# Yoshiki172/Deep-Learning-based-RGBA-Image-Compression-with-Masked-Window-based-Attention

Hardware: AMD Instinct MI355X
Metric: MPixels/sec encode+decode, 256×256 RGBA batch; bpp & PSNR parity vs reference (higher is better)
Workload: dtype bf16; 1 GPU; AutoEncoderRGB_Journal forward encode+decode (BASELINE config 2), 256x256 RGBA; global_batch=8, per_gpu_batch=8, height=256, width=256, parallelism=replicas1, hip_graph=True, tile_cache=profiles/tune_fwd_bf16_b8_256.json

## Files before the change

### deep-learning-based-rgba-image-compression-with-masked-window-based-attention_amd/csrc/fused.hip

```cpp
#include <cstdlib>

#include "common.h"

namespace rgbac {

constexpr int kRuMaxGroups = 4;

struct RuGroup {
  const bf16_t* x; long long ldx;
  const bf16_t* w1; const bf16_t* w2; const bf16_t* w3;
  int kp1, kp2, kp3;
  const float* b1; const float* b2; const float* b3;
  bf16_t* out; long long ldo;
};
struct RuArgsDev {
  int batch, H, W, ngroups;
  int stagger;
  RuGroup g[kRuMaxGroups];
  const bf16_t* gw;
  const float* gb;
  const bf16_t* gid; long long ldid;
  unsigned* flags;
  unsigned* timeout;
};
// ... 750 lines not shown
  for (int j = 0; j < 3; ++j) b2v[j] = *reinterpret_cast<const float4*>(bs + 96 + 48 * wn + 16 * j + 4 * fq);
#pragma unroll
  for (int j = 0; j < 3; ++j) {
    const int n = 48 * wn + 16 * j + 4 * fq;
    const float4 bb = b2v[j];
#pragma unroll
    for (int i = 0; i < 4; ++i) {
      const int p = (4 * wm + i) * TX + fr;
      float v[4];
      ru_act4<RB>(v, acc2[j][i], bb);
      Elem<bf16_t>::st4(reinterpret_cast<bf16_t*>(&T2[p * TROW + n * 2]), v);
    }
  }
  RU_T(5);
  __syncthreads();
  RU_T(6);

  f32x4 acc3[6][4];
#pragma unroll
  for (int j = 0; j < 6; ++j)
#pragma unroll
    for (int i = 0; i < 4; ++i) acc3[j][i] = f32x4{0.f, 0.f, 0.f, 0.f};
  const unsigned char* const t2l = T2 + (4 * wm * TX + fr) * TROW + fq * 16;
#pragma unroll
  for (int ks = 0; ks < NK3; ++ks) {
    uint4 bv[4];
#pragma unroll
    for (int i = 0; i < 4; ++i) bv[i] = *reinterpret_cast<const uint4*>(t2l + i * TX * TROW + ks * 64);
#pragma unroll
    for (int j = 0; j < 6; ++j)
#pragma unroll
      for (int i = 0; i < 4; ++i) mma_step<bf16_t>(acc3[j][i], w3r[ks % R3][j], bv[i]);
    if (ks + R3 < NK3) {
#pragma unroll
      for (int j = 0; j < 6; ++j) w3r[ks % R3][j] = W3[(j * NK3 + ks + R3) * 64];
    }
  }
  if constexpr (RB != 0) load_res();
  float4 b3v[6];
#pragma unroll
  for (int j = 0; j < 6; ++j) b3v[j] = *reinterpret_cast<const float4*>(bs + 192 + 96 * wn + 16 * j + 4 * fq);
  __syncthreads();
#pragma unroll
  for (int i = 0; i < 4; ++i) {
    const int p = (4 * wm + i) * TX + fr;
#pragma unroll
    for (int j = 0; j < 6; ++j) {
      const int n = 96 * wn + 16 * j + 4 * fq;
      const float4 bb = b3v[j];
      const uint2 rr = res[i][j];
      float v[4];
      v[0] = acc3[j][i][0] + bb.x + bf2f(rr.x & 0xFFFF);
      v[1] = acc3[j][i][1] + bb.y + bf2f(rr.x >> 16);
      v[2] = acc3[j][i][2] + bb.z + bf2f(rr.y & 0xFFFF);
      v[3] = acc3[j][i][3] + bb.w + bf2f(rr.y >> 16);
      if (!RB) gelu4_fast(v);
      Elem<bf16_t>::st4(reinterpret_cast<bf16_t*>(OT + p * ORW + n * 2), v);
    }
  }
  __syncthreads();
  if constexpr (GATE) {
    if (blockIdx.z == 1) {
      ru_gate_tile(args, OT, tile, b, y0, x0, wn, wm, fr, fq, lane);
      return;
    }
  }
#pragma unroll
  for (int u = 0; u < TY * TX * 24 / NTH; ++u) {
    const int c = tid + NTH * u, p = c / 24, q = c - (c / 24) * 24;
    const long long pix = (long long)(b * args.H + y0 + p / TX) * args.W + x0 + p % TX;
    const uint4 v = *reinterpret_cast<const uint4*>(OT + p * ORW + q * 16);
    if constexpr (GATE) st16_wt(g.out + pix * g.ldo + q * 8, v);
    else *reinterpret_cast<uint4*>(g.out + pix * g.ldo + q * 8) = v;
  }
  if constexpr (GATE) {
    asm volatile("s_waitcnt vmcnt(0)" ::: "memory");
    __syncthreads();
    if (tid == 0)
      __hip_atomic_store(&args.flags[tile], 1u, __ATOMIC_RELAXED, __HIP_MEMORY_SCOPE_AGENT);
  }
  RU_T(7);
}
#undef RU_T

}

using namespace rgbac;

#ifdef RGBAC_RU_TIMING
extern "C" int rgbac_debug_ru_times(unsigned long long* host, int nblocks) {
  if (nblocks > 8192) nblocks = 8192;
  if (hipMemcpyFromSymbol(host, HIP_SYMBOL(g_ru_t), (size_t)nblocks * 16 * 8) != hipSuccess) return 1;
  return hipMemcpyFromSymbol(host + (size_t)nblocks * 16, HIP_SYMBOL(g_ru_w), (size_t)nblocks * 2 * 8) ==
                 hipSuccess ? 0 : 1;
}
#endif

extern "C" int rgbac_residual_unit(const rgbac_ru_args* args, int ngroups, void* stream) {
  return rgbac_residual_unit_ex(args, ngroups, 0, stream);
}

extern "C" int rgbac_residual_unit_ex(const rgbac_ru_args* args, int ngroups, int kind,
                                      void* stream) {
  RGBAC_REQUIRE(args != nullptr && ngroups >= 1 && ngroups <= kRuMaxGroups, "groups");
  const rgbac_ru_args* a = args;
  RGBAC_REQUIRE(a->dtype == RGBAC_BF16, "the fused residual unit is bf16 only");
  RGBAC_REQUIRE(kind == 0 || kind == 1, "kind: 0 = ResidualUnit, 1 = ResBlock");
  RGBAC_REQUIRE(a->channels == 192 || a->channels == 80, "fused units support C = 192 or 80");
  RGBAC_REQUIRE(a->batch > 0 && a->h > 0 && a->w > 0 && a->h % 8 == 0 && a->w % 8 == 0,
                "H and W must be positive multiples of 8");
  RuArgsDev d{};
  d.batch = a->batch; d.H = a->h; d.W = a->w; d.ngroups = ngroups;
  static const int stagger_env = [] {
    const char* e = getenv("RGBAC_RU_STAGGER");
    return e ? atoi(e) : 0;
  }();
  d.stagger = stagger_env;
  for (int i = 0; i < ngroups; ++i) {
    const rgbac_ru_args* q = &args[i];
    RGBAC_REQUIRE(q->dtype == a->dtype && q->channels == a->channels && q->batch == a->batch &&
                      q->h == a->h && q->w == a->w, "grouped units must share the geometry");
    RGBAC_REQUIRE(q->x && q->out && q->w1 && q->w2 && q->w3 && q->b1 && q->b2 && q->b3,
                  "null pointer");
    RGBAC_REQUIRE(q->x != q->out, "out must not alias x (the halo is read by other tiles)");
    RGBAC_REQUIRE(q->x_ldc >= a->channels && q->x_ldc % 8 == 0 && q->out_ldc >= a->channels &&
                      q->out_ldc % 4 == 0, "strides");
    if (a->channels == 192 && q->w1_kpad != 0)
      RGBAC_REQUIRE(q->w1_kpad >= 192 && q->w2_kpad >= 896 && q->w3_kpad >= 96 &&
                        q->w1_kpad % 8 == 0 && q->w2_kpad % 8 == 0 && q->w3_kpad % 8 == 0,
                    "packed weight k_pad (w1 >= 192, w2 >= 896 zero-padded, w3 >= 96)");
    RGBAC_REQUIRE(((uintptr_t)q->x % 16) == 0 && ((uintptr_t)q->w1 % 16) == 0 &&
                      ((uintptr_t)q->w2 % 16) == 0 && ((uintptr_t)q->w3 % 16) == 0,
                  "16-byte alignment");
    RuGroup& g = d.g[i];
    g.x = (const bf16_t*)q->x; g.ldx = q->x_ldc;
    g.w1 = (const bf16_t*)q->w1; g.w2 = (const bf16_t*)q->w2; g.w3 = (const bf16_t*)q->w3;
    g.kp1 = q->w1_kpad; g.kp2 = q->w2_kpad; g.kp3 = q->w3_kpad;
    g.b1 = q->b1; g.b2 = q->b2; g.b3 = q->b3;
    g.out = (bf16_t*)q->out; g.ldo = q->out_ldc;
  }
  hipStream_t st = reinterpret_cast<hipStream_t>(stream);
  if (a->channels == 80) {
    const long long tiles = (long long)a->batch * (a->h / 8) * (a->w / 8);
    RGBAC_REQUIRE(tiles < (1ll << 31), "too many tiles");
    const int ncu = device_cus();
    long long gx = ncu / ngroups;
    if (gx < 1) gx = 1;
    const char* dual_env = getenv("RGBAC_RU_SMALL_DUAL");
    const bool dual = (tiles > gx && !(dual_env && dual_env[0] == '0')) || (dual_env && dual_env[0] == '2');
    if (dual) {
      if (gx > (tiles + 1) / 2) gx = (tiles + 1) / 2;
      if (kind) hipLaunchKernelGGL((ru_small_kernel<1, 2>), dim3((unsigned)gx, 1, ngroups), dim3(512), 0, st, d);
      else hipLaunchKernelGGL((ru_small_kernel<0, 2>), dim3((unsigned)gx, 1, ngroups), dim3(512), 0, st, d);
    } else {
      if (gx > tiles) gx = tiles;
      if (kind) hipLaunchKernelGGL((ru_small_kernel<1, 1>), dim3((unsigned)gx, 1, ngroups), dim3(256), 0, st, d);
      else hipLaunchKernelGGL((ru_small_kernel<0, 1>), dim3((unsigned)gx, 1, ngroups), dim3(256), 0, st, d);
    }
    return check_launch("ru_small_kernel");
  }
  if (a->w1_kpad == 0) {
    RGBAC_REQUIRE(a->h % 8 == 0 && a->w % 16 == 0, "the streamed unit needs H % 8 == 0, W % 16 == 0");
    for (int i = 0; i < ngroups; ++i)
      RGBAC_REQUIRE(args[i].w1_kpad == 0 && args[i].w2_kpad == 0 && args[i].w3_kpad == 0 &&
                        ((uintptr_t)args[i].b1 % 16) == 0 && ((uintptr_t)args[i].b2 % 16) == 0 &&
                        ((uintptr_t)args[i].b3 % 16) == 0 && args[i].out_ldc % 8 == 0 &&
                        ((uintptr_t)args[i].out % 16) == 0,
                    "grouped units must all be fragment-major (16-B aligned biases and out rows)");
    const long long tiles = (long long)a->batch * (a->h / 8) * (a->w / 16);
    RGBAC_REQUIRE(tiles < (1ll << 31), "too many tiles");
    for (int i = 0; i < ngroups; ++i)
      RGBAC_REQUIRE((long long)a->batch * a->h * a->w * args[i].x_ldc < (1ll << 31),
                    "the streamed unit addresses x with 32-bit element offsets");
    if (kind) hipLaunchKernelGGL((ru_stream_kernel<1, 8>), dim3((unsigned)tiles, 1, ngroups), dim3(256), 0, st, d);
    else hipLaunchKernelGGL((ru_stream_kernel<0, 8>), dim3((unsigned)tiles, 1, ngroups), dim3(256), 0, st, d);
    return check_launch("ru_stream_kernel");
  }
  static const int wide_env = [] {
    const char* e = getenv("RGBAC_RU_TILE");
    return (e && e[0] == '8') ? 0 : 1;
  }();
  if (wide_env && a->w % 16 == 0) {
    const long long tiles = (long long)a->batch * (a->h / 8) * (a->w / 16);
    RGBAC_REQUIRE(tiles < (1ll << 31), "too many tiles");
    if (kind) hipLaunchKernelGGL((ru_fused_kernel<192, 96, 8, 16, 2, 1>), dim3((unsigned)tiles, 1, ngroups),
                                 dim3(256), 0, st, d);
    else hipLaunchKernelGGL((ru_fused_kernel<192, 96, 8, 16, 2>), dim3((unsigned)tiles, 1, ngroups),
                            dim3(256), 0, st, d);
  } else {
    const long long tiles = (long long)a->batch * (a->h / 8) * (a->w / 8);
    RGBAC_REQUIRE(tiles < (1ll << 31), "too many tiles");
    if (kind) hipLaunchKernelGGL((ru_fused_kernel<192, 96, 8, 8, 3, 1>), dim3((unsigned)tiles, 1, ngroups),
                                 dim3(256), 0, st, d);
    else hipLaunchKernelGGL((ru_fused_kernel<192, 96, 8, 8, 3>), dim3((unsigned)tiles, 1, ngroups),
                            dim3(256), 0, st, d);
  }
  return check_launch("ru_fused_kernel");
}

extern "C" int rgbac_residual_unit_gate(const rgbac_ru_args* args, const void* gate_w,
                                        const float* gate_b, const void* ident, int64_t ident_ldc,
                                        uint32_t* flags, int64_t nflags, void* stream) {
  RGBAC_REQUIRE(args != nullptr && gate_w && gate_b && ident && flags, "null pointer");
  const rgbac_ru_args* a = args;
  RGBAC_REQUIRE(a->dtype == RGBAC_BF16 && a->channels == 192,
                "the gated unit pair is bf16, C = 192 only");
  RGBAC_REQUIRE(a->batch > 0 && a->h > 0 && a->w > 0 && a->h % 8 == 0 && a->w % 16 == 0,
                "the gated unit pair needs H % 8 == 0, W % 16 == 0");
  const long long tiles = (long long)a->batch * (a->h / 8) * (a->w / 16);
  RGBAC_REQUIRE(tiles < (1ll << 31) && nflags >= tiles + 1,
                "flags: one zeroed word per 8 x 16 tile plus the timeout word (the last)");
  RGBAC_REQUIRE(((uintptr_t)flags % 4) == 0 && ((uintptr_t)gate_w % 16) == 0 &&
                    ((uintptr_t)gate_b % 16) == 0 && ((uintptr_t)ident % 8) == 0 &&
                    ident_ldc >= 192 && ident_ldc % 4 == 0,
                "gate operand alignment / stride");
  RGBAC_REQUIRE((long long)a->batch * a->h * a->w * ident_ldc < (1ll << 31) ||
                    ident_ldc > 0, "identity stride");
  RuArgsDev d{};
  d.batch = a->batch; d.H = a->h; d.W = a->w; d.ngroups = 2;
  for (int i = 0; i < 2; ++i) {
    const rgbac_ru_args* q = &args[i];
    RGBAC_REQUIRE(q->dtype == a->dtype && q->channels == 192 && q->batch == a->batch &&
                      q->h == a->h && q->w == a->w, "both units must share the geometry");
    RGBAC_REQUIRE(q->x && q->out && q->w1 && q->w2 && q->w3 && q->b1 && q->b2 && q->b3,
                  "null pointer");
    RGBAC_REQUIRE(q->x != q->out && q->out != ident, "out must alias neither x nor the identity");
    RGBAC_REQUIRE(q->w1_kpad == 0 && q->w2_kpad == 0 && q->w3_kpad == 0,
                  "fragment-major packs only (the streamed unit)");
    RGBAC_REQUIRE(q->x_ldc >= 192 && q->x_ldc % 8 == 0 && q->out_ldc >= 192 &&
                      q->out_ldc % 8 == 0, "strides");
    RGBAC_REQUIRE(((uintptr_t)q->x % 16) == 0 && ((uintptr_t)q->w1 % 16) == 0 &&
                      ((uintptr_t)q->w2 % 16) == 0 && ((uintptr_t)q->w3 % 16) == 0 &&
                      ((uintptr_t)q->b1 % 16) == 0 && ((uintptr_t)q->b2 % 16) == 0 &&
                      ((uintptr_t)q->b3 % 16) == 0 && ((uintptr_t)q->out % 16) == 0,
                  "16-byte alignment");
    RGBAC_REQUIRE((long long)a->batch * a->h * a->w * q->x_ldc < (1ll << 31),
                  "the streamed unit addresses x with 32-bit element offsets");
    RuGroup& g = d.g[i];
    g.x = (const bf16_t*)q->x; g.ldx = q->x_ldc;
    g.w1 = (const bf16_t*)q->w1; g.w2 = (const bf16_t*)q->w2; g.w3 = (const bf16_t*)q->w3;
    g.b1 = q->b1; g.b2 = q->b2; g.b3 = q->b3;
    g.out = (bf16_t*)q->out; g.ldo = q->out_ldc;
  }
  d.gw = (const bf16_t*)gate_w; d.gb = gate_b;
  d.gid = (const bf16_t*)ident; d.ldid = ident_ldc;
  d.flags = flags; d.timeout = flags + (nflags - 1);
  hipStream_t st = reinterpret_cast<hipStream_t>(stream);
  hipLaunchKernelGGL((ru_stream_kernel<0, 8, true>), dim3((unsigned)tiles, 1, 2), dim3(256), 0, st, d);
  return check_launch("ru_stream_kernel");
}
```

### deep-learning-based-rgba-image-compression-with-masked-window-based-attention_amd/rgbac/_lib.py

```python
import ctypes
import os

import torch

_HERE = os.path.dirname(os.path.abspath(__file__))
LIB_PATH = os.environ.get("RGBAC_LIB_PATH") or os.path.join(_HERE, "librgbac_hip.so")

F32, BF16 = 0, 1
ACT = dict(none=0, gelu=1, relu=2, lrelu=3, tanh_half=4, gate=5, gdn=6, igdn=7, masksel=8,
           gauss=9, sqbwd=10, dgelu=11, dlrelu=12)
CONV, CONVT_S2, SUBPEL2 = 0, 1, 2


class Src(ctypes.Structure):
    _fields_ = [("ptr", ctypes.c_void_p), ("ldc", ctypes.c_int64),
                ("channels", ctypes.c_int32), ("_pad", ctypes.c_int32)]


class ConvArgs(ctypes.Structure):
    _fields_ = [
        ("dtype", ctypes.c_int32), ("mode", ctypes.c_int32),
        ("batch", ctypes.c_int32), ("in_h", ctypes.c_int32), ("in_w", ctypes.c_int32),
        ("ksize", ctypes.c_int32), ("stride", ctypes.c_int32),
        ("nsrc", ctypes.c_int32), ("src", Src * 3),
# ... 5 lines not shown
        ("out_coff", ctypes.c_int32), ("act", ctypes.c_int32),
        ("act_param", ctypes.c_float), ("square_input", ctypes.c_int32),
        ("res0", ctypes.c_void_p), ("res0_ldc", ctypes.c_int64),
        ("res1", ctypes.c_void_p), ("res1_ldc", ctypes.c_int64),
        ("res2", ctypes.c_void_p), ("res2_ldc", ctypes.c_int64),
        ("sel", ctypes.c_void_p),
        ("tile", ctypes.c_int32), ("ksplit", ctypes.c_int32),
        ("workspace", ctypes.c_void_p),
        ("aux0", ctypes.c_void_p), ("aux1", ctypes.c_void_p), ("partial", ctypes.c_void_p),
        ("zout", ctypes.c_void_p), ("zout_ldc", ctypes.c_int64),
        ("tile_counters", ctypes.c_void_p),
    ]


class WgradArgs(ctypes.Structure):
    _fields_ = [
        ("dtype", ctypes.c_int32),
        ("batch", ctypes.c_int32), ("grid_h", ctypes.c_int32), ("grid_w", ctypes.c_int32),
        ("g", ctypes.c_void_p), ("g_ldc", ctypes.c_int64), ("g_channels", ctypes.c_int32),
        ("in_h", ctypes.c_int32), ("in_w", ctypes.c_int32), ("ksize", ctypes.c_int32),
        ("stride", ctypes.c_int32), ("pad", ctypes.c_int32),
        ("nsrc", ctypes.c_int32), ("cin_pad", ctypes.c_int32),
        ("src", Src * 3),
        ("square_input", ctypes.c_int32),
        ("n_pad", ctypes.c_int32), ("k_pad", ctypes.c_int32),
        ("nsplit", ctypes.c_int32),
        ("partial", ctypes.c_void_p), ("bias_partial", ctypes.c_void_p),
    ]


class RuArgs(ctypes.Structure):
    _fields_ = [
        ("dtype", ctypes.c_int32), ("channels", ctypes.c_int32), ("batch", ctypes.c_int32),
        ("h", ctypes.c_int32), ("w", ctypes.c_int32), ("_pad0", ctypes.c_int32),
        ("x", ctypes.c_void_p), ("x_ldc", ctypes.c_int64),
        ("w1", ctypes.c_void_p), ("w2", ctypes.c_void_p), ("w3", ctypes.c_void_p),
        ("w1_kpad", ctypes.c_int32), ("w2_kpad", ctypes.c_int32), ("w3_kpad", ctypes.c_int32),
        ("_pad1", ctypes.c_int32),
        ("b1", ctypes.c_void_p), ("b2", ctypes.c_void_p), ("b3", ctypes.c_void_p),
        ("out", ctypes.c_void_p), ("out_ldc", ctypes.c_int64),
    ]


class RansDecoderState(ctypes.Structure):
    _fields_ = [("state", ctypes.c_uint64), ("data", ctypes.c_void_p), ("size", ctypes.c_int64),
                ("pos", ctypes.c_int64)]


_VP, _I32, _I64, _F = ctypes.c_void_p, ctypes.c_int, ctypes.c_int64, ctypes.c_float
_D = ctypes.c_double
SIGNATURES = {
    "rgbac_abi_version": [],
    "rgbac_last_error": [],
    "rgbac_conv2d": [ctypes.POINTER(ConvArgs), _VP],
    "rgbac_conv_num_tiles": [],
    "rgbac_conv_tile_weight_layout": [ctypes.c_int],
    "rgbac_conv2d_grouped": [ctypes.c_void_p, _I32, _VP],
    "rgbac_conv2d_grouped_part": [ctypes.c_void_p, _I32, _I32, _VP],
    "rgbac_conv_max_groups": [],
    "rgbac_timer_create": [ctypes.POINTER(ctypes.c_void_p)],
    "rgbac_timer_record": [_VP, _VP],
    "rgbac_timer_elapsed_ms": [_VP, _VP, ctypes.POINTER(ctypes.c_float)],
    "rgbac_timer_destroy": [_VP],
    "rgbac_winattn_core": [_I32, _I32, _I32, _I32, _I32, _I32, _I32, _I32, _I32, _F,
                           _VP, _I64, _VP, _VP, _VP, _I64, _VP, _VP],
    "rgbac_winattn_core_ex": [_I32, _I32, _I32, _I32, _I32, _I32, _I32, _I32, _I32, _F,
                              _VP, _I64, _VP, _VP, _VP, _I64, _VP, _VP, _I32, _I32, _VP],
    "rgbac_gaussian_slice": [_I32, _I64, _I32, _VP, _I64, _VP, _I64, _VP, _I64, _VP,
                             _VP, _I64, _VP, _VP, _VP],
    "rgbac_eb_forward": [_I32, _I64, _I32, _VP, _I64, _VP, _VP, _VP, _I64, _VP, _VP, _VP],
    "rgbac_reduce_blocks": [_I64],
    "rgbac_finalize": [_I32, _I32, _I32, _I32, _I32, _I32, _VP, _VP, _I64, _VP, _VP, _I32,
                       _VP, _I32, _VP, _VP, _VP],
    "rgbac_finalize_blocks": [_I32, _I32],
    "rgbac_finalize_ex": [_I32, _I32, _I32, _I32, _I32, _I32, _VP, _VP, _I64, _VP, _VP, _I32,
                          _VP, _I32, _VP, _VP, _VP, _VP],
    "rgbac_forward_prologue": [_I32, _I32, _I32, _I32, _I32, _VP, _VP, _I64, _VP, _I32, _VP,
                               _I32, _VP, _VP, _I64, _VP],
    "rgbac_mask_pyramid": [_I32, _I32, _I32, _VP, _I32, _VP, _I32, _VP, _VP],
    "rgbac_nchw_to_nhwc": [_I32, _I32, _I32, _I32, _I32, _VP, _VP, _I64, _VP],
    "rgbac_nhwc_to_nchw": [_I32, _I32, _I32, _I32, _I32, _VP, _I64, _VP, _VP],
    "rgbac_residual_unit": [_VP, _I32, _VP],
    "rgbac_residual_unit_ex": [_VP, _I32, _I32, _VP],
    "rgbac_residual_unit_gate": [_VP, _VP, _VP, _VP, _I64, _VP, _I64, _VP],
    "rgbac_stem_gdn": [_I32, _I32, _I32, _VP, _I64, _VP, _I32, _VP, _VP, _I32, _VP, _I32, _VP,
                       _I64, _VP],
    "rgbac_winattn_block": [_I32, _I32, _I32, _I32, _I32, _F, _VP, _I64, _VP, _VP, _VP, _VP, _VP,
                            _VP, _I64, _VP, _I64, _VP],
    "rgbac_winattn_block_workspace": [_I32, _I32, _I32],
    "rgbac_gdn_reparam": [_I32, _I32, _VP, _VP, _F, _F, _F, _VP, _VP, _VP],
    "rgbac_gdn_reparam_bwd": [_I32, _I32, _VP, _VP, _F, _F, _VP, _VP, _VP, _VP, _I32, _VP],
    "rgbac_eb_params": [_I32, _VP, _VP, _VP],
    "rgbac_eb_params_bwd": [_I32, _VP, _VP, _VP, _I32, _VP],
    "rgbac_winattn_block_ws4": [_I32, _I32, _I32, _I32, _I32, _F, _VP, _I64, _VP, _VP, _VP, _VP,
                                _VP, _VP, _VP, _I64, _VP],
    "rgbac_rgba_augment": [_I32, _VP, _I32, _I32, _I32, _VP, _VP, _VP, _VP, _VP],
    "rgbac_dse_block": [_I32, _I32, _I32, _I32, _I32, _F, _VP, _I64, _VP, _I64, _VP, _I32, _VP, _VP,
                        _I32, _VP, _VP, _I32, _VP, _VP, _I32, _VP, _VP, _I64, _VP],
    "rgbac_act_bwd": [_I32, _I32, _F, _I64, _I32, _VP, _I64, _VP, _I64, _VP, _I64, _VP, _VP,
                      _I64, _VP, _I64, _VP],
    "rgbac_conv_wgrad": [ctypes.POINTER(WgradArgs), _VP],
    "rgbac_wgrad_reduce": [_I64, _VP, _VP, _I32, _I64, _VP, _I32, _VP, _I32, _VP, _I32, _VP],
    "rgbac_wgrad_reduce_multi": [_I32, _VP, _VP],
    "rgbac_winattn_core_bwd": [_I32, _I32, _I32, _I32, _I32, _I32, _I32, _I32, _I32, _F, _VP,
                               _I64, _VP, _VP, _VP, _I64, _VP, _I64, _I32, _VP, _VP],
    "rgbac_winattn_core_bwd_ex": [_I32, _I32, _I32, _I32, _I32, _I32, _I32, _I32, _I32, _F,
                                  _VP, _I64, _VP, _VP, _VP, _I64, _VP, _I64, _I32, _VP, _VP,
                                  _I32, _VP],
    "rgbac_relpos_bwd": [_I32, _I32, _I32, _VP, _VP, _VP, _VP, _VP, _VP],
    "rgbac_gaussian_bwd": [_I32, _I64, _I32, _VP, _I64, _VP, _I64, _VP, _I64, _VP, _VP, _VP,
                           _I64, _VP, _I64, _VP, _I64, _VP, _I64, _VP],
    "rgbac_eb_bwd": [_I32, _I64, _I32, _VP, _I64, _VP, _VP, _VP, _VP, _I64, _VP, _I64, _VP, _VP],
    "rgbac_mse_bwd": [_I32, _I32, _I32, _I32, _I32, _I32, _VP, _VP, _I64, _VP, _VP, _VP, _VP,
                      _I64, _VP],
    "rgbac_adam_clamp": [_I64, _VP, _VP, _VP, _VP, _D, _D, _D, _D, _I64, _F, _F, _VP],
    "rgbac_adam_clamp_dstep": [_I64, _VP, _VP, _VP, _VP, _D, _D, _D, _D, _VP, _F, _F, _VP],
    "rgbac_pixel_shuffle": [_I32, _I32, _I32, _I32, _I32, _I32, _VP, _I64, _VP, _I64, _VP],
    "rgbac_channel_copy": [_I32, _I64, _I32, _VP, _I64, _I32, _VP, _I64, _I32, _VP],
    "rgbac_channel_copy_multi": [_I32, _I64, _I32, _VP, _VP],
    "rgbac_channel_copy_multi_ex": [_I32, _I64, _I32, _VP, _VP],
    "rgbac_weight_gather": [_I32, _I64, _VP, _VP, _VP, _VP],
    "rgbac_weight_gather_multi": [_I32, _VP, _VP, _I64, _VP],
    "rgbac_weight_repack_multi": [_I32, _VP, _VP, _I64, _VP],
    "rgbac_colsum": [_I32, _I64, _I32, _VP, _I64, _I32, _VP, _VP],
    "rgbac_sum_partials": [_I32, _I32, _VP, _VP, _VP],
    "rgbac_gauss_code": [_I32, _I32, _I32, _I32, _I32, _I32, _VP, _I64, _VP, _I64, _VP, _I32, _F,
                         _VP, _VP, _VP, _I64, _VP],
    "rgbac_eb_code": [_I32, _I32, _I32, _I32, _I32, _I32, _VP, _I64, _VP, _VP, _VP, _I64, _VP],
    "rgbac_alpha_recon": [_I32, _I32, _I32, _I32, _VP, _VP, _VP, _VP, _VP],
    "rgbac_rgba_finish": [_I64, _VP, _VP, _VP, _VP, _VP, _VP, _VP, _VP, _VP],
    "rgbac_ssim_level": [_I32, _I32, _I32, _I32, _I32, _VP, _VP, _VP, _F, _F, _VP, _VP, _VP, _VP],
    "rgbac_avgpool2": [_I32, _I32, _I32, _VP, _VP, _VP],
    "rgbac_msssim_combine": [_I32, _I32, _VP, _VP, _VP, _VP, _VP, _VP],
    "rgbac_masked_apply": [_I32, _I32, _I32, _I32, _I32, _VP, _VP, _VP, _VP, _VP, _VP, _VP],
    "rgbac_masked_ssim_level": [_I32, _I32, _I32, _I32, _I32, _I32, _VP, _VP, _VP, _VP, _F, _F,
                                _VP, _VP, _VP, _VP],
    "rgbac_masked_msssim_combine": [_I32, _I32, _I32, _VP, _VP, _VP, _VP, _VP, _VP],
    "rgbac_ssim_level_bwd": [_I32, _I32, _I32, _I32, _I32, _VP, _VP, _VP, _F, _F, _VP, _VP, _VP,
                             _VP, _VP, _VP, _VP],
    "rgbac_masked_ssim_level_bwd": [_I32, _I32, _I32, _I32, _I32, _I32, _VP, _VP, _VP, _VP, _F, _F,
                                    _VP, _VP, _VP, _I32, _VP, _VP, _VP, _VP, _VP],
    "rgbac_msssim_combine_bwd": [_I32, _I32, _VP, _VP, _VP, _VP, _I32, _VP, _VP],
    "rgbac_masked_msssim_combine_bwd": [_I32, _I32, _I32, _VP, _VP, _VP, _VP, _I32, _VP, _VP],
    "rgbac_pmf_to_quantized_cdf": [_VP, _I32, _I32, _VP],
    "rgbac_rans_encoder_create": [ctypes.POINTER(ctypes.c_void_p)],
    "rgbac_rans_encoder_destroy": [_VP],
    "rgbac_rans_encoder_put": [_VP, _VP, _VP, _I64, _VP, _I32, _VP, _VP, _I32],
    "rgbac_comm_load": [ctypes.c_char_p],
    "rgbac_comm_unique_id": [_VP],
    "rgbac_comm_init": [_VP, _I32, _I32, _I32, ctypes.POINTER(ctypes.c_void_p)],
    "rgbac_comm_allreduce_sum": [_VP, _I32, _VP, _I64, _VP],
    "rgbac_comm_destroy": [_VP],
    "rgbac_comm_count": [_VP, ctypes.POINTER(ctypes.c_int)],
    "rgbac_comm_async_error": [_VP, ctypes.POINTER(ctypes.c_int)],
    "rgbac_comm_abort": [_VP],
    "rgbac_rans_encoder_bound": [_VP],
    "rgbac_rans_encoder_flush": [_VP, _VP, _I64, ctypes.POINTER(ctypes.c_int64)],
    "rgbac_rans_decoder_init": [ctypes.POINTER(RansDecoderState), _VP, _I64],
    "rgbac_rans_decode": [ctypes.POINTER(RansDecoderState), _VP, _I64, _VP, _I32, _VP, _VP, _I32,
                          _VP],
    "rgbac_rans_chunk_sizes": [_VP, _VP, _I64, _I64, _VP, _VP, _I64, _I32, _VP, _I32, _VP, _VP,
                               _I32, _VP, _VP, _VP],
    "rgbac_rans_chunk_encode": [_VP, _VP, _I64, _I64, _VP, _VP, _I64, _I32, _VP, _I32, _VP, _VP,
                                _I32, _VP, _VP, _VP, _I64, _VP, _VP],
    "rgbac_rans_chunk_decode": [_VP, _I64, _VP, _VP, _VP, _I64, _I64, _VP, _VP, _I64, _I32, _VP,
                                _I32, _VP, _VP, _I32, _VP, _VP, _VP],
# ... 58 lines not shown
```

### deep-learning-based-rgba-image-compression-with-masked-window-based-attention_amd/rgbac/layers/Masked_Attention.py

```python
import ctypes
import os

import torch
import torch.nn as nn

from .. import _lib
from .. import runtime as rt
from ._blocks import conv1x1, conv3x3
from .masked_win_attention import WinBasedAttention, needs_grad


class ResidualUnit(nn.Module):

    def __init__(self, N):
        super().__init__()
        self.conv = nn.Sequential(conv1x1(N, N // 2), nn.GELU(), conv3x3(N // 2, N // 2),
                                  nn.GELU(), conv1x1(N // 2, N))
        self.relu = nn.GELU()

    def nhwc(self, x):
        return run_residual_units([(self, x)])[0]

    def forward(self, x):
        rt.check_gpu(x)
# ... 116 lines not shown
        dual_env = os.environ.get("RGBAC_RU_SMALL_DUAL", "")
        dual = (tiles > max(1, ncu // len(units)) and dual_env != "0") or dual_env == "2"
        kname = f"ru_small_kernel<{kind}, {2 if dual else 1}>"
    elif stream:
        kname = f"ru_stream_kernel<{kind}, 8, false>"
    else:
        kname = f"ru_fused_kernel<{C}, {C // 2}>"
    rt.timed(kname, flops, 2 * npix * len(units) * 2 * C,
             lambda: _lib.call("rgbac_residual_unit_ex", ctypes.addressof(arr), len(units), kind,
                               _lib.stream_ptr(x0.t.device)),
             f"{kname} kind{kind} g{len(units)} C{C} {x0.H}x{x0.W} B{x0.B}")
    return outs


GATE_FUSED = os.environ.get("RGBAC_GATE_FUSED", "1") != "0"


def gate_pack(conv):
    key = (rt.PARAM_GEN, conv.weight._version, conv.weight.data_ptr(), conv.bias._version,
           conv.bias.data_ptr())
    ent = conv.__dict__.get("_rgbac_gate_pack")
    if ent is None or ent[0] != key:
        with torch.no_grad():
            kfn = lambda ks, l, e: 32 * ks + 8 * (l >> 4) + e
            pw = _frag_pack(conv.weight.float().reshape(192, 192), 12, 6, kfn)
            pb = conv.bias.float().contiguous().clone()
        conv.__dict__["_rgbac_gate_pack"] = (key, (pw, pb))
        ent = conv.__dict__["_rgbac_gate_pack"]
    return ent[1]


_FLAGS = {}


def gate_flags(dev, n):
    buf = _FLAGS.get(dev)
    if buf is None or buf.numel() < n:
        if torch.cuda.is_current_stream_capturing():
            return None
        buf = torch.zeros(max(n, 1 << 16), dtype=torch.int32, device=dev)
        _FLAGS[dev] = buf
    return buf


def gated_ok(block, a, b, x):
    return (GATE_FUSED and STREAM and _fused_ok([(block.conv_a[2], a), (block.conv_b[2], b)]) and
            a.C == 192 and a.W % 16 == 0 and x.ldc % 8 == 0 and
            block.conv_b[3].weight.shape == (192, 192, 1, 1))


def run_last_units_gated(block, a, b, x):
    ntiles = a.B * (a.H // 8) * (a.W // 16)
    flags = gate_flags(a.t.device, ntiles + 1)
    if flags is None:
        return None
    arr = (_lib.RuArgs * 2)()
    keep = []
    outs = []
    for i, (u, t) in enumerate(((block.conv_a[2], a), (block.conv_b[2], b))):
        c1, c2, c3 = u.conv[0], u.conv[2], u.conv[4]
        p1, p2, p3, b1, b2, b3 = wide_unit_packs(c1, c2, c3)
        o = rt.new_feat(t.B, t.H, t.W, t.C, t.t.dtype, t.t.device)
        r = arr[i]
        r.dtype, r.channels, r.batch, r.h, r.w = _lib.BF16, t.C, t.B, t.H, t.W
        r.x, r.x_ldc = t.ptr(), t.ldc
        r.w1, r.w2, r.w3 = p1.data_ptr(), p2.data_ptr(), p3.data_ptr()
        r.w1_kpad = r.w2_kpad = r.w3_kpad = 0
        r.b1, r.b2, r.b3 = b1.data_ptr(), b2.data_ptr(), b3.data_ptr()
        r.out, r.out_ldc = o.ptr(), o.ldc
        keep.append((p1, p2, p3, b1, b2, b3))
        outs.append(o)
    gw, gb = gate_pack(block.conv_b[3])
    npix = a.B * a.H * a.W
    C = 192
    flops = 2.0 * npix * (2 * (C * C // 2 * 2 + 9 * (C // 2) ** 2) + C * C)
    rt.timed("ru_stream_kernel<0, 8, true>", flops, 2 * npix * 6 * C,
             lambda: _lib.call("rgbac_residual_unit_gate", ctypes.addressof(arr), gw.data_ptr(),
                               gb.data_ptr(), x.ptr(), x.ldc, flags.data_ptr(), flags.numel(),
                               _lib.stream_ptr(a.t.device)),
             f"ru_stream_kernel<0, 8, true> gate C{C} {a.H}x{a.W} B{a.B}")
    return outs[1]


def run_residual_units_fused(pairs):
    return run_bottlenecks_fused([((u.conv[0], u.conv[2], u.conv[4]), x) for u, x in pairs], 0)


def run_residual_units(pairs):
    if _fused_ok(pairs):
        return run_residual_units_fused(pairs)
    return run_residual_units_unfused(pairs)


def run_residual_units_unfused(pairs):
    from .TransformRGB import prep_conv
    ts = rt.launch([prep_conv(u.conv[0], [x.src()], act="gelu") for u, x in pairs])
    ts = rt.launch([prep_conv(u.conv[2], [t.src()], act="gelu") for (u, _), t in zip(pairs, ts)])
    return rt.launch([prep_conv(u.conv[4], [t.src()], act="gelu", res0=x)
                      for (u, x), t in zip(pairs, ts)])


class Win_noShift_Attention(nn.Module):

    def __init__(self, dim, num_heads=8, window_size=8, shift_size=0):
        super().__init__()
        N = dim
        self.conv_a = nn.Sequential(ResidualUnit(N), ResidualUnit(N), ResidualUnit(N))
        self.attn = WinBasedAttention(dim=dim, num_heads=num_heads, window_size=window_size,
                                      shift_size=shift_size)
        self.conv_b = nn.Sequential(ResidualUnit(N), ResidualUnit(N), ResidualUnit(N),
                                    conv1x1(N, N))

    def nhwc(self, x, mask):
        b = self.attn.nhwc(x, mask)
        a = x
        for k in range(2):
            a, b = run_residual_units([(self.conv_a[k], a), (self.conv_b[k], b)])
        if gated_ok(self, a, b, x):
            out = run_last_units_gated(self, a, b, x)
            if out is not None:
                return out
        a, b = run_residual_units([(self.conv_a[2], a), (self.conv_b[2], b)])
        pk = rt.packed(self.conv_b[3], x.t.dtype, rt.segs_of(b.src()))
        return rt.conv(pk, [b.src()], act="gate", res1=a, res2=x)

    def forward(self, x, mask):
        rt.check_gpu(x, mask)
        if needs_grad(self, x):
            from ..train_forward import attention_block_t, layer_t
            return layer_t(lambda f: attention_block_t(self, f, mask), x)
        with torch.no_grad():
            return rt.to_nchw(self.nhwc(rt.to_nhwc(x, torch.float32), mask))
```

### include/rgbac.h

```cpp
#ifndef RGBAC_H_
#define RGBAC_H_

#include <stdint.h>

#ifdef __cplusplus
extern "C" {
#endif

#define RGBAC_ABI_VERSION 2

enum rgbac_status {
  RGBAC_OK = 0,
  RGBAC_E_ARG = -1,
  RGBAC_E_DTYPE = -2,
  RGBAC_E_LAUNCH = -3,
};

enum rgbac_dtype { RGBAC_F32 = 0, RGBAC_BF16 = 1 };

enum rgbac_act {
  RGBAC_ACT_NONE = 0,
  RGBAC_ACT_GELU = 1,
  RGBAC_ACT_RELU = 2,
  RGBAC_ACT_LRELU = 3,
// ... 44 lines not shown
  int32_t tile;
  int32_t ksplit;
  void* workspace;
  const float* aux0;
  float* aux1;
  double* partial;
  void* zout;
  int64_t zout_ldc;
  int32_t* tile_counters;
} rgbac_conv_args;

int rgbac_abi_version(void);
const char* rgbac_last_error(void);

int rgbac_conv2d(const rgbac_conv_args* args, void* stream);
int rgbac_conv_num_tiles(void);
int rgbac_conv_tile_weight_layout(int tile);

int rgbac_conv2d_grouped(const rgbac_conv_args* args, int ngroups, void* stream);
int rgbac_conv_max_groups(void);

int rgbac_conv2d_grouped_part(const rgbac_conv_args* args, int ngroups, int part, void* stream);

int rgbac_winattn_core(int dtype, int batch, int h, int w, int channels,
                       int heads, int ws, int shift, int masked, float scale,
                       const void* qkv, int64_t ldq, const float* alpha,
                       const float* bias, void* out, int64_t ldo, uint8_t* sel,
                       void* stream);
int rgbac_winattn_core_ex(int dtype, int batch, int h, int w, int channels,
                          int heads, int ws, int shift, int masked, float scale,
                          const void* qkv, int64_t ldq, const float* alpha,
                          const float* bias, void* out, int64_t ldo, uint8_t* sel,
                          const float* amask, int amask_nw, int hpb, void* stream);

int rgbac_gaussian_slice(int dtype, int64_t npix, int nch,
                         const void* y, int64_t ldy, const void* mu, int64_t ldmu,
                         const void* scale, int64_t lds, const float* noise,
                         void* out_hat, int64_t ldh, float* lik, double* partial,
                         void* stream);

int rgbac_eb_forward(int dtype, int64_t npix, int channels, const void* z,
                     int64_t ldz, const float* params, const float* noise,
                     void* z_hat, int64_t ldh, float* lik, double* partial,
                     void* stream);

int rgbac_reduce_blocks(int64_t n);

int rgbac_finalize(int dtype, int mode, int batch, int cx, int h, int w,
                   const float* x, const void* x_hat, int64_t ldh,
                   const float* mask, const double* ybits, int ny,
                   const double* zbits, int nz, double* scratch, float* out,
                   void* stream);
int rgbac_finalize_blocks(int h, int w);
int rgbac_finalize_ex(int dtype, int mode, int batch, int cx, int h, int w,
                      const float* x, const void* x_hat, int64_t ldh,
                      const float* mask, const double* ybits, int ny,
                      const double* zbits, int nz, double* scratch, float* out,
                      float* x_hat_nchw, void* stream);
int rgbac_forward_prologue(int dtype, int batch, int c, int h, int w, const float* x,
                           void* xf, int64_t ldc, const float* alpha, int round255,
                           float* rounded, int levels, float* const* outs,
                           double* zero, int64_t nzero, void* stream);

int rgbac_mask_pyramid(int batch, int h, int w, const float* alpha, int round255,
                       float* rounded, int levels, float* const* outs,
                       void* stream);

int rgbac_nchw_to_nhwc(int dtype, int batch, int c, int h, int w,
                       const float* src, void* dst, int64_t ldc, void* stream);
int rgbac_nhwc_to_nchw(int dtype, int batch, int c, int h, int w,
                       const void* src, int64_t ldc, float* dst, void* stream);


typedef struct rgbac_ru_args {
  int32_t dtype, channels, batch, h, w, _pad0;
  const void* x; int64_t x_ldc;
  const void* w1; const void* w2; const void* w3;
  int32_t w1_kpad, w2_kpad, w3_kpad, _pad1;
  const float* b1; const float* b2; const float* b3;
  void* out; int64_t out_ldc;
} rgbac_ru_args;
int rgbac_residual_unit(const rgbac_ru_args* args, int ngroups, void* stream);
int rgbac_residual_unit_ex(const rgbac_ru_args* args, int ngroups, int kind, void* stream);
int rgbac_residual_unit_gate(const rgbac_ru_args* args, const void* gate_w,
                             const float* gate_b, const void* ident, int64_t ident_ldc,
                             uint32_t* flags, int64_t nflags, void* stream);


int rgbac_act_bwd(int dtype, int act, float act_param, int64_t npix, int channels,
                  const void* dy, int64_t ldy, const void* z, int64_t ldz, const void* res1,
                  int64_t ld1, const uint8_t* sel, void* dz, int64_t lddz, void* dres1,
                  int64_t lddr1, void* stream);

typedef struct rgbac_wgrad_args {
  int32_t dtype;
  int32_t batch, grid_h, grid_w;
  const void* g; int64_t g_ldc; int32_t g_channels;
  int32_t in_h, in_w, ksize, stride, pad;
  int32_t nsrc; int32_t cin_pad;
  rgbac_src src[3];
  int32_t square_input;
  int32_t n_pad, k_pad;
  int32_t nsplit;
  float* partial;
  float* bias_partial;
} rgbac_wgrad_args;
int rgbac_conv_wgrad(const rgbac_wgrad_args* args, void* stream);

int rgbac_wgrad_reduce(int64_t nslot, const int32_t* fmap, const float* partial, int nsplit,
                       int64_t slab, float* dw, int nbias, const float* bias_partial, int n_pad,
                       float* db, int accumulate, void* stream);

int rgbac_wgrad_reduce_multi(int ntasks, const int64_t* tasks, void* stream);

int rgbac_winattn_core_bwd(int dtype, int batch, int h, int w, int channels, int heads, int ws,
                           int shift, int masked, float scale, const void* qkv, int64_t ldq,
                           const float* alpha, const float* bias, const void* dout, int64_t ldo,
                           void* dqkv, int64_t lddq, int nblk, float* bias_partial,
                           void* stream);
int rgbac_winattn_core_bwd_ex(int dtype, int batch, int h, int w, int channels, int heads,
                              int ws, int shift, int masked, float scale, const void* qkv,
                              int64_t ldq, const float* alpha, const float* bias,
                              const void* dout, int64_t ldo, void* dqkv, int64_t lddq, int nblk,
                              float* bias_partial, const float* amask, int amask_nw,
                              void* stream);
int rgbac_relpos_bwd(int nblk, int heads, int ws, const float* bias_partial,
                     const int32_t* csr_off, const int32_t* csr_ij, float* dense, float* dtable,
                     void* stream);

int rgbac_gaussian_bwd(int dtype, int64_t npix, int nch, const void* y, int64_t ldy,
                       const void* mu, int64_t ldmu, const void* scale, int64_t lds,
                       const float* noise, const float* gbits, const void* dhat, int64_t lddh,
                       void* dy, int64_t lddy, void* dmu, int64_t lddmu, void* dscale,
                       int64_t lddsc, void* stream);

int rgbac_eb_bwd(int dtype, int64_t npix, int channels, const void* z, int64_t ldz,
                 const float* params, const float* noise, const float* gbits, const void* dzhat,
                 int64_t lddh, void* dz, int64_t lddz, float* dparams, void* stream);

int rgbac_mse_bwd(int dtype, int mode, int batch, int cx, int h, int w, const float* x,
                  const void* x_hat, int64_t ldh, const float* mask, const double* scratch,
                  const float* gmse, void* dx_hat, int64_t lddx, void* stream);

int rgbac_adam_clamp(int64_t n, float* param, float* grad, float* exp_avg, float* exp_avg_sq,
                     double lr, double beta1, double beta2, double eps, int64_t step,
                     float clip, float grad_scale, void* stream);

int rgbac_adam_clamp_dstep(int64_t n, float* param, float* grad, float* exp_avg,
                           float* exp_avg_sq, double lr, double beta1, double beta2, double eps,
                           int64_t* step_dev, float clip, float grad_scale, void* stream);

int rgbac_pixel_shuffle(int dtype, int dir, int batch, int h, int w, int c, const void* in,
                        int64_t ldi, void* out, int64_t ldo, void* stream);
int rgbac_channel_copy(int dtype, int64_t npix, int channels, const void* src, int64_t lds,
                       int scoff, void* dst, int64_t ldd, int dcoff, void* stream);
int rgbac_channel_copy_multi(int dtype, int64_t npix, int ntasks, const int64_t* desc,
                             void* stream);

int rgbac_channel_copy_multi_ex(int dtype, int64_t npix, int ntasks, const int64_t* desc,
                                void* stream);

int rgbac_weight_gather(int dtype, int64_t n, const float* src, const int32_t* idx, void* dst,
                        void* stream);

int rgbac_weight_gather_multi(int ntask, const int64_t* tasks, const int64_t* blk0, int64_t nblk,
                              void* stream);
// ... 166 lines not shown
```

Measured before the change: 323.1 MPix/s.

## Fuse three chained residual units into one halo-tiled kernel for C=80

Adds a kernel that runs three consecutive residual units in a single launch per 8x8 tile. It loads a 14x14 halo once and keeps intermediates in LDS, prefetching the next unit's weights while the current one computes. This removes the global round-trips and launches between units in the C=80 attention blocks. In exchange it recomputes the overlapping halo and uses a large LDS footprint, which allows one 1024-thread block per CU.

```diff
diff --git a/deep-learning-based-rgba-image-compression-with-masked-window-based-attention_amd/csrc/fused.hip b/deep-learning-based-rgba-image-compression-with-masked-window-based-attention_amd/csrc/fused.hip
--- a/deep-learning-based-rgba-image-compression-with-masked-window-based-attention_amd/csrc/fused.hip
+++ b/deep-learning-based-rgba-image-compression-with-masked-window-based-attention_amd/csrc/fused.hip
@@ -856,6 +856,238 @@
   RU_T(7);
 }
 #undef RU_T
+
+struct RuChainUnit {
+  const bf16_t* w1; const bf16_t* w2; const bf16_t* w3;
+  const float* b1; const float* b2; const float* b3;
+};
+struct RuChainGroup {
+  const bf16_t* x; long long ldx;
+  bf16_t* out; long long ldo;
+  RuChainUnit u[3];
+};
+struct RuChainArgs {
+  int batch, H, W, ngroups;
+  RuChainGroup g[kRuMaxGroups];
+};
+namespace ruc {
+constexpr int NU = 3;
+constexpr int NW = 16, NT = 64 * NW;
+constexpr int XS = 14, NX = XS * XS;
+constexpr int XROW = 160;
+constexpr int W1B = rus::W1F * 1024, W2B = rus::W2F * 1024, W3B = rus::W3F * 1024;
+constexpr int OFF_W1 = 0, OFF_W2 = W1B, OFF_W3 = W1B + W2B;
+constexpr int OFF_X = OFF_W3 + 2 * W3B;
+constexpr int OFF_T1 = OFF_X + NX * XROW;
+constexpr int OFF_T2 = OFF_T1 + NX * 128;
+constexpr int OFF_B = OFF_T2 + 144 * 128;
+constexpr int NB = 48 + 48 + 80;
+constexpr int LDS = OFF_B + NU * NB * 4;
+constexpr int W2_MIN = rus::W2F / NW;
+static_assert(LDS <= 160 * 1024, "LDS budget");
+static_assert(OFF_X % 16 == 0 && OFF_T1 % 16 == 0 && OFF_T2 % 16 == 0 && OFF_B % 16 == 0, "alignment");
+}
+
+__device__ __forceinline__ void ruc_dma(const bf16_t* src, uint32_t lds, int nf, int wave, int lane) {
+  for (int pc = wave; pc < nf; pc += ruc::NW)
+    ru_dma16(reinterpret_cast<const uint4*>(src) + pc * 64 + lane, lds + (uint32_t)pc * 1024u);
+}
+
+template <int K>
+__device__ __forceinline__ void ruc_unit(unsigned char* sm, const RuChainArgs& args,
+                                         const RuChainGroup& g, int wave, int lane, int b, int y0,
+                                         int x0) {
+  using namespace ruc;
+  constexpr int S1 = XS - 2 * K, S2 = S1 - 2;
+  constexpr int N1 = S1 * S1, N2 = S2 * S2;
+  constexpr int NF1 = (N1 + 15) / 16, NF2 = (N2 + 15) / 16;
+  static_assert(NF1 <= NW && NF2 <= NW, "one fragment per wave and stage");
+  constexpr bool LAST = K == NU - 1;
+  const uint4* const W1 = reinterpret_cast<const uint4*>(sm + OFF_W1);
+  const uint4* const W2 = reinterpret_cast<const uint4*>(sm + OFF_W2);
+  const uint4* const W3 = reinterpret_cast<const uint4*>(sm + OFF_W3 + (K & 1) * W3B);
+  unsigned char* const X = sm + OFF_X;
+  unsigned char* const T1b = sm + OFF_T1;
+  unsigned char* const T2b = sm + OFF_T2;
+  const uint4* const T1 = reinterpret_cast<const uint4*>(T1b);
+  const uint4* const T2 = reinterpret_cast<const uint4*>(T2b);
+  const float* const bs = reinterpret_cast<const float*>(sm + OFF_B) + K * NB;
+  const uint32_t lbase = __builtin_amdgcn_readfirstlane((uint32_t)(size_t)(ru_lptr_t)sm);
+  const int n = lane & 15, q = lane >> 4;
+
+  if (wave < NF1) {
+    const int hp = 16 * wave + n;
+    const bool ok = hp < N1;
+    const int hc = ok ? hp : 0;
+    const int ry = hc / S1, rx = hc - ry * S1;
+    const int xi = (ry + K) * XS + rx + K;
+    const int iy = y0 - 3 + ry + K, ix = x0 - 3 + rx + K;
+    const bool in = iy >= 0 && iy < args.H && ix >= 0 && ix < args.W;
+    f32x4 acc[3];
+#pragma unroll
+    for (int tt = 0; tt < 3; ++tt) acc[tt] = f32x4{0.f, 0.f, 0.f, 0.f};
+#pragma unroll
+    for (int ks = 0; ks < 3; ++ks) {
+      const int c8 = 4 * ks + q;
+      const uint4 bv = c8 < 10 ? *reinterpret_cast<const uint4*>(X + xi * XROW + c8 * 16)
+                               : make_uint4(0, 0, 0, 0);
+#pragma unroll
+      for (int tt = 0; tt < 3; ++tt) mma_step<bf16_t>(acc[tt], W1[(tt * 3 + ks) * 64 + lane], bv);
+    }
+    if (ok) {
+#pragma unroll
+      for (int tt = 0; tt < 3; ++tt) {
+        const int c0 = 16 * tt + 4 * q;
+        float v[4];
+#pragma unroll
+        for (int r = 0; r < 4; ++r) v[r] = acc[tt][r] + bs[c0 + r];
+        gelu4_fast(v);
+#pragma unroll
+        for (int r = 0; r < 4; ++r) v[r] = in ? v[r] : 0.0f;
+        *reinterpret_cast<uint2*>(T1b + hp * 128 + (((c0 >> 3) ^ (hp & 7)) << 4) + 2 * (c0 & 7)) =
+            make_uint2(pack_bf16x2(v[0], v[1]), pack_bf16x2(v[2], v[3]));
+      }
+    }
+  }
+  asm volatile("s_waitcnt vmcnt(0)" ::: "memory");
+  __syncthreads();
+  if constexpr (!LAST) {
+    ruc_dma(g.u[K + 1].w3, lbase + OFF_W3 + ((K + 1) & 1) * W3B, rus::W3F, wave, lane);
+    ruc_dma(g.u[K + 1].w1, lbase + OFF_W1, rus::W1F, wave, lane);
+  }
+
+  const int p = 16 * wave + n;
+  const bool pok = p < N2;
+  const int pc = pok ? p : 0;
+  const int py = pc / S2, px = pc - py * S2;
+
+  if (wave < NF2) {
+    f32x4 acc[3];
+#pragma unroll
+    for (int tt = 0; tt < 3; ++tt) acc[tt] = f32x4{0.f, 0.f, 0.f, 0.f};
+#pragma unroll
+    for (int kk = 0; kk < 18; ++kk) {
+      const int tap = kk >> 1, c8 = 4 * (kk & 1) + q;
+      const int hp = (py + tap / 3) * S1 + px + tap % 3;
+      const uint4 bv = T1[hp * 8 + (c8 ^ (hp & 7))];
+#pragma unroll
+      for (int tt = 0; tt < 3; ++tt) mma_step<bf16_t>(acc[tt], W2[(tt * 18 + kk) * 64 + lane], bv);
+    }
+    if (pok) {
+#pragma unroll
+      for (int tt = 0; tt < 3; ++tt) {
+        const int c0 = 16 * tt + 4 * q;
+        float v[4];
+#pragma unroll
+        for (int r = 0; r < 4; ++r) v[r] = acc[tt][r] + bs[48 + c0 + r];
+        gelu4_fast(v);
+        *reinterpret_cast<uint2*>(T2b + p * 128 + (((c0 >> 3) ^ (p & 7)) << 4) + 2 * (c0 & 7)) =
+            make_uint2(pack_bf16x2(v[0], v[1]), pack_bf16x2(v[2], v[3]));
+      }
+    }
+  }
+  __syncthreads();
+  if constexpr (!LAST) ruc_dma(g.u[K + 1].w2, lbase + OFF_W2, rus::W2F, wave, lane);
+
+  if (wave < NF2) {
+    f32x4 acc[5];
+#pragma unroll
+    for (int tt = 0; tt < 5; ++tt) acc[tt] = f32x4{0.f, 0.f, 0.f, 0.f};
+#pragma unroll
+    for (int ks = 0; ks < 2; ++ks) {
+      const int c8 = 4 * ks + q;
+      const uint4 bv = T2[pc * 8 + (c8 ^ (pc & 7))];
+#pragma unroll
+      for (int tt = 0; tt < 5; ++tt) mma_step<bf16_t>(acc[tt], W3[(tt * 2 + ks) * 64 + lane], bv);
+    }
+    if (pok) {
+      unsigned char* const xrow = X + ((py + K + 1) * XS + px + K + 1) * XROW;
+      bf16_t* orow = nullptr;
+      if constexpr (LAST)
+        orow = g.out + ((long long)(b * args.H + y0 + py) * args.W + x0 + px) * g.ldo;
+#pragma unroll
+      for (int tt = 0; tt < 5; ++tt) {
+        const int c0 = 16 * tt + 4 * q;
+        const uint2 rx = *reinterpret_cast<const uint2*>(xrow + 2 * c0);
+        const float res[4] = {bf2f(rx.x & 0xFFFF), bf2f(rx.x >> 16), bf2f(rx.y & 0xFFFF),
+                              bf2f(rx.y >> 16)};
+        float v[4];
+#pragma unroll
+        for (int r = 0; r < 4; ++r) v[r] = acc[tt][r] + bs[96 + c0 + r] + res[r];
+        gelu4_fast(v);
+        if constexpr (LAST) Elem<bf16_t>::st4(orow + c0, v);
+        else
+          *reinterpret_cast<uint2*>(xrow + 2 * c0) =
+              make_uint2(pack_bf16x2(v[0], v[1]), pack_bf16x2(v[2], v[3]));
+      }
+    }
+  }
+  if constexpr (!LAST) {
+    asm volatile("s_waitcnt vmcnt(%0)" ::"n"(W2_MIN) : "memory");
+    __syncthreads();
+  }
+}
+
+__global__ void __launch_bounds__(64 * ruc::NW, 1) ru_chain_kernel(const RuChainArgs args) {
+  using namespace ruc;
+  extern __shared__ __attribute__((aligned(16))) unsigned char ruc_sm[];
+  unsigned char* const sm = ruc_sm;
+  const RuChainGroup& g = args.g[blockIdx.z];
+  const int tid = threadIdx.x, lane = tid & 63;
+  const int wave = __builtin_amdgcn_readfirstlane(tid >> 6);
+  const int tx_n = args.W / 8, ty_n = args.H / 8;
+  const int tc = blockIdx.x;
+  const int tx = tc % tx_n, ty = (tc / tx_n) % ty_n, b = tc / (tx_n * ty_n);
+  const int y0 = ty * 8, x0 = tx * 8;
+
+  {
+    const uint32_t lbase = __builtin_amdgcn_readfirstlane((uint32_t)(size_t)(ru_lptr_t)sm);
+    ruc_dma(g.u[0].w1, lbase + OFF_W1, rus::W1F, wave, lane);
+    ruc_dma(g.u[0].w3, lbase + OFF_W3, rus::W3F, wave, lane);
+    ruc_dma(g.u[0].w2, lbase + OFF_W2, rus::W2F, wave, lane);
+  }
+  {
+    constexpr int NJ = (NX * 10 + NT - 1) / NT;
+    uint4 xv[NJ];
+#pragma unroll
+    for (int j = 0; j < NJ; ++j) {
+      const int e = tid + NT * j;
+      const int pix = e / 10, c = e - 10 * pix;
+      const int ay = pix / XS, ax = pix - ay * XS;
+      const int iy = y0 - 3 + ay, ix = x0 - 3 + ax;
+      const bool in = e < NX * 10 && iy >= 0 && iy < args.H && ix >= 0 && ix < args.W;
+      xv[j] = in ? *reinterpret_cast<const uint4*>(
+                       g.x + ((long long)(b * args.H + iy) * args.W + ix) * g.ldx + 8 * c)
+                 : make_uint4(0, 0, 0, 0);
+    }
+#pragma unroll
+    for (int j = 0; j < NJ; ++j) {
+      const int e = tid + NT * j;
+      if (e < NX * 10) *reinterpret_cast<uint4*>(sm + OFF_X + e * 16) = xv[j];
+    }
+  }
+  {
+    float* const bs = reinterpret_cast<float*>(sm + OFF_B);
+    for (int e = tid; e < NU * NB; e += NT) {
+      const RuChainUnit& u = g.u[e / NB];
+      const int k = e % NB;
+      bs[e] = k < 48 ? u.b1[k] : k < 96 ? u.b2[k - 48] : u.b3[k - 96];
+    }
+  }
+  for (int e = tid; e < (NX + 144) * 2; e += NT) {
+    const int p = e >> 1, c = 6 + (e & 1);
+    uint4* const T1 = reinterpret_cast<uint4*>(sm + OFF_T1);
+    uint4* const T2 = reinterpret_cast<uint4*>(sm + OFF_T2);
+    if (p < NX) T1[p * 8 + (c ^ (p & 7))] = make_uint4(0, 0, 0, 0);
+    else T2[(p - NX) * 8 + (c ^ ((p - NX) & 7))] = make_uint4(0, 0, 0, 0);
+  }
+  asm volatile("s_waitcnt vmcnt(0)" ::: "memory");
+  __syncthreads();
+
+  ruc_unit<0>(sm, args, g, wave, lane, b, y0, x0);
+  ruc_unit<1>(sm, args, g, wave, lane, b, y0, x0);
+  ruc_unit<2>(sm, args, g, wave, lane, b, y0, x0);
+}
 
 }
 
@@ -970,6 +1202,48 @@
                             dim3(256), 0, st, d);
   }
   return check_launch("ru_fused_kernel");
+}
+
+extern "C" int rgbac_residual_unit_chain(const rgbac_ru_args* args, int ngroups, int nunits,
+                                         void* stream) {
+  RGBAC_REQUIRE(args != nullptr && ngroups >= 1 && ngroups <= kRuMaxGroups, "groups");
+  RGBAC_REQUIRE(nunits == ruc::NU, "a chain is three units");
+  const rgbac_ru_args* a = args;
+  RGBAC_REQUIRE(a->dtype == RGBAC_BF16 && a->channels == 80, "the unit chain is bf16, C = 80 only");
+  RGBAC_REQUIRE(a->batch > 0 && a->h > 0 && a->w > 0 && a->h % 8 == 0 && a->w % 8 == 0,
+                "H and W must be positive multiples of 8");
+  const long long tiles = (long long)a->batch * (a->h / 8) * (a->w / 8);
+  RGBAC_REQUIRE(tiles < (1ll << 31), "too many tiles");
+  RuChainArgs d{};
+  d.batch = a->batch; d.H = a->h; d.W = a->w; d.ngroups = ngroups;
+  for (int i = 0; i < ngroups; ++i) {
+    const rgbac_ru_args* first = &args[i * nunits];
+    const rgbac_ru_args* last = &args[i * nunits + nunits - 1];
+    RGBAC_REQUIRE(first->x && last->out && first->x != last->out,
+                  "x / out: null, or out aliases x (the halo is read by other tiles)");
+    RGBAC_REQUIRE(first->x_ldc >= 80 && first->x_ldc % 8 == 0 && last->out_ldc >= 80 &&
+                      last->out_ldc % 4 == 0 && ((uintptr_t)first->x % 16) == 0 &&
+                      ((uintptr_t)last->out % 8) == 0, "strides / alignment of x and out");
+    RuChainGroup& g = d.g[i];
+    g.x = (const bf16_t*)first->x; g.ldx = first->x_ldc;
+    g.out = (bf16_t*)last->out; g.ldo = last->out_ldc;
+    for (int k = 0; k < nunits; ++k) {
+      const rgbac_ru_args* q = &args[i * nunits + k];
+      RGBAC_REQUIRE(q->dtype == a->dtype && q->channels == 80 && q->batch == a->batch &&
+                        q->h == a->h && q->w == a->w, "chained units must share the geometry");
+      RGBAC_REQUIRE(q->w1 && q->w2 && q->w3 && q->b1 && q->b2 && q->b3, "null pointer");
+      RGBAC_REQUIRE(((uintptr_t)q->w1 % 16) == 0 && ((uintptr_t)q->w2 % 16) == 0 &&
+                        ((uintptr_t)q->w3 % 16) == 0, "16-byte alignment");
+      RuChainUnit& u = g.u[k];
+      u.w1 = (const bf16_t*)q->w1; u.w2 = (const bf16_t*)q->w2; u.w3 = (const bf16_t*)q->w3;
+      u.b1 = q->b1; u.b2 = q->b2; u.b3 = q->b3;
+    }
+  }
+  static unsigned long long attr = 0;
+  lds_optin(reinterpret_cast<const void*>(ru_chain_kernel), ruc::LDS, &attr);
+  hipStream_t st = reinterpret_cast<hipStream_t>(stream);
+  hipLaunchKernelGGL(ru_chain_kernel, dim3((unsigned)tiles, 1, ngroups), dim3(ruc::NT), ruc::LDS, st, d);
+  return check_launch("ru_chain_kernel");
 }
 
 extern "C" int rgbac_residual_unit_gate(const rgbac_ru_args* args, const void* gate_w,
diff --git a/deep-learning-based-rgba-image-compression-with-masked-window-based-attention_amd/rgbac/_lib.py b/deep-learning-based-rgba-image-compression-with-masked-window-based-attention_amd/rgbac/_lib.py
--- a/deep-learning-based-rgba-image-compression-with-masked-window-based-attention_amd/rgbac/_lib.py
+++ b/deep-learning-based-rgba-image-compression-with-masked-window-based-attention_amd/rgbac/_lib.py
@@ -111,6 +111,7 @@
     "rgbac_nhwc_to_nchw": [_I32, _I32, _I32, _I32, _I32, _VP, _I64, _VP, _VP],
     "rgbac_residual_unit": [_VP, _I32, _VP],
     "rgbac_residual_unit_ex": [_VP, _I32, _I32, _VP],
+    "rgbac_residual_unit_chain": [_VP, _I32, _I32, _VP],
     "rgbac_residual_unit_gate": [_VP, _VP, _VP, _VP, _I64, _VP, _I64, _VP],
     "rgbac_stem_gdn": [_I32, _I32, _I32, _VP, _I64, _VP, _I32, _VP, _VP, _I32, _VP, _I32, _VP,
                        _I64, _VP],
diff --git a/deep-learning-based-rgba-image-compression-with-masked-window-based-attention_amd/rgbac/layers/Masked_Attention.py b/deep-learning-based-rgba-image-compression-with-masked-window-based-attention_amd/rgbac/layers/Masked_Attention.py
--- a/deep-learning-based-rgba-image-compression-with-masked-window-based-attention_amd/rgbac/layers/Masked_Attention.py
+++ b/deep-learning-based-rgba-image-compression-with-masked-window-based-attention_amd/rgbac/layers/Masked_Attention.py
@@ -222,6 +222,43 @@
     return outs[1]
 
 
+RU_CHAIN = os.environ.get("RGBAC_RU_CHAIN", "1") != "0"
+
+
+def chain_ok(block, a, b):
+    return (RU_CHAIN and FUSED and not torch.is_grad_enabled() and
+            all(t.t.dtype == torch.bfloat16 and t.C == 80 and t.H % 8 == 0 and t.W % 8 == 0 and
+                t.ldc % 8 == 0 for t in (a, b)) and
+            (a.B, a.H, a.W) == (b.B, b.H, b.W) and len(block.conv_a) == 3)
+
+
+def run_unit_chains(chains):
+    x0 = chains[0][1]
+    C, nu = x0.C, len(chains[0][0])
+    arr = (_lib.RuArgs * (len(chains) * nu))()
+    outs, keep = [], []
+    for i, (units, x) in enumerate(chains):
+        o = rt.new_feat(x.B, x.H, x.W, x.C, x.t.dtype, x.t.device)
+        for k, u in enumerate(units):
+            p1, p2, p3, b1, b2, b3 = small_unit_packs(u.conv[0], u.conv[2], u.conv[4])
+            a = arr[i * nu + k]
+            a.dtype, a.channels, a.batch, a.h, a.w = _lib.BF16, x.C, x.B, x.H, x.W
+            a.w1, a.w2, a.w3 = p1.data_ptr(), p2.data_ptr(), p3.data_ptr()
+            a.w1_kpad = a.w2_kpad = a.w3_kpad = 0
+            a.b1, a.b2, a.b3 = b1.data_ptr(), b2.data_ptr(), b3.data_ptr()
+            keep.append((p1, p2, p3, b1, b2, b3))
+        arr[i * nu].x, arr[i * nu].x_ldc = x.ptr(), x.ldc
+        arr[i * nu + nu - 1].out, arr[i * nu + nu - 1].out_ldc = o.ptr(), o.ldc
+        outs.append(o)
+    npix = x0.B * x0.H * x0.W
+    flops = 2.0 * npix * len(chains) * nu * (C * C // 2 * 2 + 9 * (C // 2) ** 2)
+    rt.timed("ru_chain_kernel", flops, 2 * npix * len(chains) * 2 * C,
+             lambda: _lib.call("rgbac_residual_unit_chain", ctypes.addressof(arr), len(chains), nu,
+                               _lib.stream_ptr(x0.t.device)),
+             f"ru_chain_kernel g{len(chains)} x{nu} C{C} {x0.H}x{x0.W} B{x0.B}")
+    return outs
+
+
 def run_residual_units_fused(pairs):
     return run_bottlenecks_fused([((u.conv[0], u.conv[2], u.conv[4]), x) for u, x in pairs], 0)
 
@@ -254,13 +291,16 @@
     def nhwc(self, x, mask):
         b = self.attn.nhwc(x, mask)
         a = x
-        for k in range(2):
-            a, b = run_residual_units([(self.conv_a[k], a), (self.conv_b[k], b)])
-        if gated_ok(self, a, b, x):
-            out = run_last_units_gated(self, a, b, x)
-            if out is not None:
-                return out
-        a, b = run_residual_units([(self.conv_a[2], a), (self.conv_b[2], b)])
+        if chain_ok(self, a, b):
+            a, b = run_unit_chains([(list(self.conv_a), a), (list(self.conv_b)[:3], b)])
+        else:
+            for k in range(2):
+                a, b = run_residual_units([(self.conv_a[k], a), (self.conv_b[k], b)])
+            if gated_ok(self, a, b, x):
+                out = run_last_units_gated(self, a, b, x)
+                if out is not None:
+                    return out
+            a, b = run_residual_units([(self.conv_a[2], a), (self.conv_b[2], b)])
         pk = rt.packed(self.conv_b[3], x.t.dtype, rt.segs_of(b.src()))
         return rt.conv(pk, [b.src()], act="gate", res1=a, res2=x)
 
diff --git a/include/rgbac.h b/include/rgbac.h
--- a/include/rgbac.h
+++ b/include/rgbac.h
@@ -150,6 +150,7 @@
 } rgbac_ru_args;
 int rgbac_residual_unit(const rgbac_ru_args* args, int ngroups, void* stream);
 int rgbac_residual_unit_ex(const rgbac_ru_args* args, int ngroups, int kind, void* stream);
+int rgbac_residual_unit_chain(const rgbac_ru_args* args, int ngroups, int nunits, void* stream);
 int rgbac_residual_unit_gate(const rgbac_ru_args* args, const void* gate_w,
                              const float* gate_b, const void* ident, int64_t ident_ldc,
                              uint32_t* flags, int64_t nflags, void* stream);
```

After: 321.6 MPix/s. Within noise of the previous version (-0.5%).
